# PasaLab/marlin

Measured on NVIDIA B200. Metric: fp64 dense multiply throughput (2*N^3 flop), 16384x16384 BlockMatrix 2x2 grid, higher is better.
Workload: dtype f64

## Files before the change

### include/marlin_b200.h

```cpp
#ifndef MARLIN_B200_H
#define MARLIN_B200_H

#include <stdint.h>
#include <stddef.h>

#ifdef __cplusplus
extern "C" {
#endif
#if defined(__GNUC__)
#pragma GCC visibility push(default)
#endif

#define MB_OK                 0
#define MB_ERR_INVALID_ARG   -1
#define MB_ERR_DIM_MISMATCH  -2
#define MB_ERR_UNSUPPORTED   -3
#define MB_ERR_CUDA          -4
#define MB_ERR_OOM           -5
#define MB_ERR_EMPTY         -6

typedef enum { MB_F64 = 0, MB_BF16 = 1, MB_F32 = 2 } mb_dtype;

typedef struct mb_ctx   mb_ctx;
typedef struct mb_block mb_block;
// ... 51 lines not shown
int32_t mb_block_sum(mb_ctx* ctx, const mb_block* A, double* sum_out);

int32_t mb_block_gemv(mb_ctx* ctx, const mb_block* A, const mb_block* x, mb_block* y, int32_t accumulate);
int32_t mb_block_dot(mb_ctx* ctx, const mb_block* x, const mb_block* y, double* dot_out);
int32_t mb_block_ger(mb_ctx* ctx, const mb_block* x, const mb_block* y, mb_block* out);

int32_t mb_block_lu(mb_ctx* ctx, mb_block* A, int32_t* perm_out);
int32_t mb_block_cholesky(mb_ctx* ctx, mb_block* A);
int32_t mb_block_inverse(mb_ctx* ctx, const mb_block* A, mb_block* out);
int32_t mb_block_trsm(mb_ctx* ctx, const mb_block* T, int32_t lower, int32_t unit_diagonal, mb_block* B);

int32_t mb_fill_uniform(mb_ctx* ctx, mb_block* blk, int64_t partition_seed, int64_t first,
                        double lo, double hi, int32_t row_major);
int64_t mb_hash_seed(int64_t seed);
int32_t mb_partition_seeds(int64_t seed, int32_t num_partitions, int64_t* seeds_out);

int32_t mb_choose_split(int64_t m, int64_t k, int64_t n, int32_t cores, int32_t out_mkn[3]);
int32_t mb_choose_strategy(int64_t a_rows, int64_t a_cols, int64_t b_cols, int32_t cores,
                           int32_t broadcast_threshold_mb, int32_t other_is_block,
                           int32_t* strategy, int32_t out_mkn[3]);
int32_t mb_mult_partition(int32_t i, int32_t j, int32_t kk, int32_t m, int32_t k, int32_t n);
int32_t mb_elem_partition(int32_t row, int32_t col, int32_t blks_by_col);
int32_t mb_block_len(int64_t total, int32_t parts, int32_t* block_len, int32_t* actual_parts);

int32_t mb_matmul_blocked(mb_ctx* ctx, mb_block* const* A_tiles, mb_block* const* B_tiles,
                          int32_t m, int32_t k, int32_t n, mb_block* const* C_tiles);
int32_t mb_matmul_blocked_subset(mb_ctx* ctx, mb_block* const* A_tiles, mb_block* const* B_tiles,
                                 int32_t m, int32_t k, int32_t n, mb_block* const* C_tiles,
                                 const int32_t* c_ids, int32_t num_c);

int32_t mb_matmul_blocked_host(mb_ctx* ctx, const double* const* A_host, const double* const* B_host,
                               int32_t m, int32_t k, int32_t n, const int32_t* row_len, const int32_t* k_len,
                               const int32_t* col_len, double* const* C_host);

int32_t mb_matmul_rowsharded(mb_ctx* ctx, const mb_block* A_rows, const mb_block* B, mb_block* C_rows);
int32_t mb_matmul_rowsharded_host(mb_ctx* ctx, const double* A_host, int64_t rows, int32_t k, const double* B_host,
                                  int32_t n, double* C_host);

int32_t mb_ipc_export(mb_ctx* ctx, const void* device_ptr, uint8_t handle_out[64], int64_t* offset_out,
                      int64_t* alloc_bytes_out);
int32_t mb_ipc_open(mb_ctx* ctx, const uint8_t handle[64], void** base_out);
int32_t mb_ipc_close_all(mb_ctx* ctx);
int32_t mb_flags_alloc(mb_ctx* ctx, int32_t count, void** flags_out);
int32_t mb_flags_free(mb_ctx* ctx, void* flags);
int32_t mb_flag_signal(mb_ctx* ctx, void* flag, int64_t value);
int32_t mb_flag_wait(mb_ctx* ctx, const void* flag, int64_t value);
int32_t mb_memcpy_async(mb_ctx* ctx, void* dst, const void* src, int64_t bytes);

typedef struct mb_comm mb_comm;
#define MB_ERR_TIMEOUT       -7
int32_t mb_comm_init(mb_ctx* ctx, int32_t rank, int32_t world, const char* session, mb_comm** out);
int32_t mb_comm_destroy(mb_comm* comm);
int32_t mb_comm_rank(const mb_comm* comm);
int32_t mb_comm_world(const mb_comm* comm);
int32_t mb_comm_barrier(mb_comm* comm);
int32_t mb_comm_abort(mb_comm* comm);
int32_t mb_comm_check(mb_comm* comm);
int32_t mb_dist_plan(int32_t m, int32_t k, int32_t n, int32_t world, int32_t* product_rank_out, int32_t* c_owner_out);
int32_t mb_matmul_blocked_dist(mb_comm* comm, mb_block* const* A_tiles, const int32_t* a_owner,
                               mb_block* const* B_tiles, const int32_t* b_owner, int32_t m, int32_t k, int32_t n,
                               const int32_t* row_len, const int32_t* k_len, const int32_t* col_len, int32_t dtype,
                               mb_block* const* C_tiles);

int32_t mb_dist_host_homes(int32_t m, int32_t k, int32_t n, int32_t world, int32_t* a_home, int32_t* b_home);
int32_t mb_matmul_blocked_dist_host(mb_comm* comm, const double* const* A_host, const int32_t* a_home,
                                    const double* const* B_host, const int32_t* b_home, int32_t m, int32_t k, int32_t n,
// ... 30 lines not shown
```

### marlin_b200/_native.py

```python
from __future__ import annotations

import ctypes as C
import os
from pathlib import Path

MB_OK = 0
MB_ERR_INVALID_ARG = -1
MB_ERR_DIM_MISMATCH = -2
MB_ERR_UNSUPPORTED = -3
MB_ERR_CUDA = -4
MB_ERR_OOM = -5
MB_ERR_EMPTY = -6
MB_ERR_TIMEOUT = -7

MB_F64, MB_BF16, MB_F32 = 0, 1, 2

_LIB_PATH = Path(__file__).resolve().parent / "lib" / "libmarlin_b200.so"

c_ctx = C.c_void_p
c_blk = C.c_void_p
c_sp = C.c_void_p
c_i32 = C.c_int32
c_i64 = C.c_int64
c_f64 = C.c_double
# ... 24 lines not shown
    "mb_set_fp64_mode": (c_i32, [c_ctx, c_i32, c_i32]),
    "mb_dgemm_device": (c_i32, [c_ctx, C.c_char, C.c_char, c_i32, c_i32, c_i32, c_f64, C.c_void_p, c_i32,
                                C.c_void_p, c_i32, c_f64, C.c_void_p, c_i32]),
    "mb_dgemm_device_generic": (c_i32, [c_ctx, C.c_char, C.c_char, c_i32, c_i32, c_i32, c_f64, C.c_void_p, c_i32,
                                        C.c_void_p, c_i32, c_f64, C.c_void_p, c_i32]),
    "mb_dgemm_host": (c_i32, [c_ctx, C.c_char, C.c_char, c_i32, c_i32, c_i32, c_f64, C.c_void_p, c_i64, c_i32,
                              C.c_void_p, c_i64, c_i32, c_f64, C.c_void_p, c_i64, c_i32]),
    "mb_block_add": (c_i32, [c_ctx, c_blk, c_blk, c_blk]),
    "mb_block_sub": (c_i32, [c_ctx, c_blk, c_blk, c_blk]),
    "mb_block_hadamard": (c_i32, [c_ctx, c_blk, c_blk, c_blk]),
    "mb_block_axpb": (c_i32, [c_ctx, c_blk, c_f64, c_f64, c_blk]),
    "mb_block_fill": (c_i32, [c_ctx, c_blk, c_f64]),
    "mb_block_div": (c_i32, [c_ctx, c_blk, c_f64, c_i32, c_blk]),
    "mb_block_transpose": (c_i32, [c_ctx, c_blk, c_blk]),
    "mb_block_copy": (c_i32, [c_ctx, c_blk, c_blk]),
    "mb_block_sum": (c_i32, [c_ctx, c_blk, c_dp]),
    "mb_block_gemv": (c_i32, [c_ctx, c_blk, c_blk, c_blk, c_i32]),
    "mb_block_dot": (c_i32, [c_ctx, c_blk, c_blk, c_dp]),
    "mb_block_ger": (c_i32, [c_ctx, c_blk, c_blk, c_blk]),
    "mb_block_lu": (c_i32, [c_ctx, c_blk, C.POINTER(c_i32)]),
    "mb_block_cholesky": (c_i32, [c_ctx, c_blk]),
    "mb_block_inverse": (c_i32, [c_ctx, c_blk, c_blk]),
    "mb_block_trsm": (c_i32, [c_ctx, c_blk, c_i32, c_i32, c_blk]),
    "mb_fill_uniform": (c_i32, [c_ctx, c_blk, c_i64, c_i64, c_f64, c_f64, c_i32]),
    "mb_hash_seed": (c_i64, [c_i64]),
    "mb_partition_seeds": (c_i32, [c_i64, c_i32, C.POINTER(c_i64)]),
    "mb_choose_split": (c_i32, [c_i64, c_i64, c_i64, c_i32, C.POINTER(c_i32)]),
    "mb_choose_strategy": (c_i32, [c_i64, c_i64, c_i64, c_i32, c_i32, c_i32, C.POINTER(c_i32), C.POINTER(c_i32)]),
    "mb_mult_partition": (c_i32, [c_i32, c_i32, c_i32, c_i32, c_i32, c_i32]),
    "mb_elem_partition": (c_i32, [c_i32, c_i32, c_i32]),
    "mb_block_len": (c_i32, [c_i64, c_i32, C.POINTER(c_i32), C.POINTER(c_i32)]),
    "mb_matmul_blocked_host": (c_i32, [c_ctx, C.POINTER(C.c_void_p), C.POINTER(C.c_void_p), c_i32, c_i32, c_i32,
                                       C.POINTER(c_i32), C.POINTER(c_i32), C.POINTER(c_i32), C.POINTER(C.c_void_p)]),
    "mb_matmul_rowsharded": (c_i32, [c_ctx, c_blk, c_blk, c_blk]),
    "mb_matmul_rowsharded_host": (c_i32, [c_ctx, C.c_void_p, c_i64, c_i32, C.c_void_p, c_i32, C.c_void_p]),
    "mb_ipc_export": (c_i32, [c_ctx, C.c_void_p, C.c_char_p, C.POINTER(c_i64), C.POINTER(c_i64)]),
    "mb_ipc_open": (c_i32, [c_ctx, C.c_char_p, C.POINTER(C.c_void_p)]),
    "mb_ipc_close_all": (c_i32, [c_ctx]),
    "mb_flags_alloc": (c_i32, [c_ctx, c_i32, C.POINTER(C.c_void_p)]),
    "mb_flags_free": (c_i32, [c_ctx, C.c_void_p]),
    "mb_flag_signal": (c_i32, [c_ctx, C.c_void_p, c_i64]),
    "mb_flag_wait": (c_i32, [c_ctx, C.c_void_p, c_i64]),
    "mb_memcpy_async": (c_i32, [c_ctx, C.c_void_p, C.c_void_p, c_i64]),
    "mb_matmul_blocked_subset": (c_i32, [c_ctx, C.POINTER(c_blk), C.POINTER(c_blk), c_i32, c_i32, c_i32, C.POINTER(c_blk),
                                         C.POINTER(c_i32), c_i32]),
    "mb_matmul_blocked": (c_i32, [c_ctx, C.POINTER(c_blk), C.POINTER(c_blk), c_i32, c_i32, c_i32, C.POINTER(c_blk)]),
    "mb_comm_init": (c_i32, [c_ctx, c_i32, c_i32, C.c_char_p, C.POINTER(C.c_void_p)]),
    "mb_comm_destroy": (c_i32, [C.c_void_p]),
    "mb_comm_rank": (c_i32, [C.c_void_p]),
    "mb_comm_world": (c_i32, [C.c_void_p]),
    "mb_comm_barrier": (c_i32, [C.c_void_p]),
    "mb_comm_check": (c_i32, [C.c_void_p]),
    "mb_comm_abort": (c_i32, [C.c_void_p]),
    "mb_dist_plan": (c_i32, [c_i32, c_i32, c_i32, c_i32, C.POINTER(c_i32), C.POINTER(c_i32)]),
    "mb_dist_host_homes": (c_i32, [c_i32, c_i32, c_i32, c_i32, C.POINTER(c_i32), C.POINTER(c_i32)]),
    "mb_matmul_blocked_dist_host": (c_i32, [C.c_void_p, C.POINTER(C.c_void_p), C.POINTER(c_i32), C.POINTER(C.c_void_p), C.POINTER(c_i32),
                                            c_i32, c_i32, c_i32, C.POINTER(c_i32), C.POINTER(c_i32), C.POINTER(c_i32), C.POINTER(C.c_void_p)]),
    "mb_host_alloc_shared": (c_i32, [C.c_char_p, c_i64, C.POINTER(C.c_void_p)]),
    "mb_host_free_shared": (c_i32, [C.c_char_p, C.c_void_p, c_i64, c_i32]),
    "mb_matmul_blocked_dist": (c_i32, [C.c_void_p, C.POINTER(c_blk), C.POINTER(c_i32), C.POINTER(c_blk), C.POINTER(c_i32), c_i32, c_i32,
                                       c_i32, C.POINTER(c_i32), C.POINTER(c_i32), C.POINTER(c_i32), c_i32, C.POINTER(c_blk)]),
    "mb_csc_check": (c_i32, [c_i32, c_i32, C.POINTER(c_i32), C.POINTER(c_i32)]),
    "mb_spblock_upload": (c_i32, [c_ctx, c_i32, c_i32, C.POINTER(c_i32), C.POINTER(c_i32), c_dp, C.POINTER(c_sp)]),
    "mb_spblock_download": (c_i32, [c_ctx, c_sp, C.POINTER(c_i32), C.POINTER(c_i32), c_dp]),
    "mb_spblock_info": (c_i32, [c_sp, C.POINTER(c_i32), C.POINTER(c_i32), C.POINTER(c_i64)]),
    "mb_spblock_free": (c_i32, [c_ctx, c_sp]),
    "mb_spblock_copy": (c_i32, [c_ctx, c_sp, C.POINTER(c_sp)]),
# ... 59 lines not shown
```

### marlin_b200/csrc/capi.cu

```cuda
#include "../../include/marlin_b200.h"
#include "elementwise.h"
#include "gemm_f64.h"
#include "gemm_bf16.h"
#include "gemm_ozaki.h"
#include "blas12.h"
#include "factor.h"
#include "sparse.h"

#include <cuda_runtime.h>
#include <algorithm>
#include <cstdarg>
#include <cstdlib>
#include <cstdio>
#include <cstring>
#include <new>
#include <atomic>
#include <mutex>
#include <vector>

#include "internal.h"

namespace {

thread_local char g_err[512] = "";
// ... 126 lines not shown
    MB_CUDA(cudaGetDeviceProperties(&prop, device));
    if (prop.major != 10)
        return fail(MB_ERR_UNSUPPORTED, "mb_init: device %d is sm_%d%d; this library is built for sm_100a only", device,
                    prop.major, prop.minor);
    mb_ctx* ctx = new (std::nothrow) mb_ctx();
    if (!ctx) return fail(MB_ERR_OOM, "host allocation failed");
    ctx->device = device;
    ctx->num_sms = prop.multiProcessorCount;
    MB_CUDA(cudaStreamCreateWithFlags(&ctx->own_stream, cudaStreamNonBlocking));
    ctx->stream = ctx->own_stream;
    MB_CUDA(cudaMalloc(&ctx->scratch, sizeof(double) * std::max(mb::sum_scratch_doubles(), mb::dot_scratch_doubles())));
    MB_CUDA(cudaMallocHost(&ctx->host_scalar, sizeof(double)));
    MB_CUDA(cudaEventCreate(&ctx->ev0));
    MB_CUDA(cudaEventCreate(&ctx->ev1));
    *out = ctx;
    return MB_OK;
}

int32_t mb_shutdown(mb_ctx* ctx) {
    if (!ctx) return MB_OK;
    cudaSetDevice(ctx->device);
    cudaStreamSynchronize(ctx->stream);
    if (ctx->scratch) cudaFree(ctx->scratch);
    if (ctx->vec_ws) cudaFree(ctx->vec_ws);
    if (ctx->int_ws) cudaFree(ctx->int_ws);
    if (ctx->int_host) cudaFreeHost(ctx->int_host);
    if (ctx->host_scalar) cudaFreeHost(ctx->host_scalar);
    if (ctx->ev0) cudaEventDestroy(ctx->ev0);
    if (ctx->ev1) cudaEventDestroy(ctx->ev1);
    if (ctx->own_stream) cudaStreamDestroy(ctx->own_stream);
    if (ctx->h2d_stream) cudaStreamDestroy(ctx->h2d_stream);
    if (ctx->d2h_stream) cudaStreamDestroy(ctx->d2h_stream);
    if (ctx->workspace) cudaFree(ctx->workspace);
    if (ctx->ozaki_ws) cudaFree(ctx->ozaki_ws);
    delete ctx;
    return MB_OK;
}

int32_t mb_set_stream(mb_ctx* ctx, void* cuda_stream) {
    if (!ctx) return fail(MB_ERR_INVALID_ARG, "null context");
    ctx->stream = static_cast<cudaStream_t>(cuda_stream);
    return MB_OK;
}

int32_t mb_reset_stream(mb_ctx* ctx) {
    if (!ctx) return fail(MB_ERR_INVALID_ARG, "null context");
    ctx->stream = ctx->own_stream;
    return MB_OK;
}

int32_t mb_synchronize(mb_ctx* ctx) {
    MB_CTX(ctx);
    MB_CUDA(cudaStreamSynchronize(ctx->stream));
    return MB_OK;
}

int64_t mb_launch_count(mb_ctx* ctx) { return ctx ? (int64_t)ctx->launches.load() : 0; }

int32_t mb_timer_start(mb_ctx* ctx) {
    MB_CTX(ctx);
    MB_LOCK(ctx);
    MB_CUDA(cudaEventRecord(ctx->ev0, ctx->stream));
    return MB_OK;
}
int32_t mb_timer_stop(mb_ctx* ctx, float* ms_out) {
    MB_CTX(ctx);
// ... 368 lines not shown
                    ++group; ns = 0; in_group = 0;
                };
                for (int kk = 0; kk < k && e == cudaSuccess; ++kk)
                    for (int k0 = 0; k0 < Ks[kk] && e == cudaSuccess;) {
                        const int len = (int)std::min<long long>(Ks[kk] - k0, kchain - in_group);
                        sa[ns] = static_cast<const char*>(Ap[kk]) + (size_t)k0 * la[kk] * 2;
                        sb[ns] = static_cast<const char*>(Bp[kk]) + (size_t)k0 * 2;
                        sla[ns] = la[kk]; slb[ns] = lb[kk]; sk[ns] = len;
                        ++ns; in_group += len; k0 += len;
                        if (in_group >= kchain || ns == 8) flush();
                    }
                flush();
            }
            if (e == cudaSuccess) { ctx->launches += launches; continue; }
            if (e != cudaErrorNotSupported) return cuda_fail(e, "gemm_bf16_segments");
            cudaGetLastError();
        }
        for (int kk = 0; kk < k; ++kk) {
            int32_t r = mb_block_gemm(ctx, A_tiles[i * k + kk], B_tiles[kk * n + j], C_tiles[id], kk > 0);
            if (r) return r;
        }
    }
    return MB_OK;
}

int32_t mb_matmul_blocked(mb_ctx* ctx, mb_block* const* A_tiles, mb_block* const* B_tiles, int32_t m, int32_t k,
                          int32_t n, mb_block* const* C_tiles) {
    if (m <= 0 || k <= 0 || n <= 0) return fail(MB_ERR_INVALID_ARG, "mb_matmul_blocked: bad argument");
    std::vector<int32_t> ids(m * n);
    for (int c = 0; c < m * n; ++c) ids[c] = c;
    return mb_matmul_blocked_subset(ctx, A_tiles, B_tiles, m, k, n, C_tiles, ids.data(), m * n);
}

int32_t mb_matmul_blocked_host(mb_ctx* ctx, const double* const* A_host, const double* const* B_host, int32_t m,
                               int32_t k, int32_t n, const int32_t* row_len, const int32_t* k_len, const int32_t* col_len,
                               double* const* C_host) {
    MB_CTX(ctx);
    MB_LOCK(ctx);
    if (!A_host || !B_host || !C_host || !row_len || !k_len || !col_len || m <= 0 || k <= 0 || n <= 0)
        return fail(MB_ERR_INVALID_ARG, "mb_matmul_blocked_host: bad argument");
    if (!ctx->h2d_stream) {
        MB_CUDA(cudaStreamCreateWithFlags(&ctx->h2d_stream, cudaStreamNonBlocking));
        MB_CUDA(cudaStreamCreateWithFlags(&ctx->d2h_stream, cudaStreamNonBlocking));
    }
    auto even = [](int x) { return (x + 1) & ~1; };
    auto slot = [](size_t bytes) { return (bytes + 255) & ~size_t(255); };
    std::vector<size_t> offA(m * k), offB(k * n), offC(m * n);
    size_t total = 0;
    for (int i = 0; i < m; ++i)
        for (int kk = 0; kk < k; ++kk) { offA[i * k + kk] = total; total += slot((size_t)even(row_len[i]) * k_len[kk] * 8); }
    for (int kk = 0; kk < k; ++kk)
        for (int j = 0; j < n; ++j) { offB[kk * n + j] = total; total += slot((size_t)even(k_len[kk]) * col_len[j] * 8); }
    for (int i = 0; i < m; ++i)
        for (int j = 0; j < n; ++j) { offC[i * n + j] = total; total += slot((size_t)even(row_len[i]) * col_len[j] * 8); }
    if (total > ctx->workspace_bytes) {
        if (ctx->workspace) { MB_CUDA(cudaDeviceSynchronize()); cudaFree(ctx->workspace); ctx->workspace = nullptr; ctx->workspace_bytes = 0; }
        MB_CUDA(cudaMalloc(&ctx->workspace, total));
        ctx->workspace_bytes = total;
    }
    char* base = static_cast<char*>(ctx->workspace);
    std::vector<cudaEvent_t> evA(m * k, nullptr), evB(k * n, nullptr), evC(m * n, nullptr);
    cudaEvent_t ev_start = nullptr, ev_done = nullptr;
    int32_t rc = MB_OK;
    cudaError_t e = cudaSuccess;
    auto upload = [&](bool isA, int idx, int rows, int cols, const double* host, size_t off, cudaEvent_t& ev) {
        if (ev || e != cudaSuccess) return;
        e = cudaEventCreateWithFlags(&ev, cudaEventDisableTiming);
        if (e != cudaSuccess) return;
        if (rows > 0 && cols > 0)
            e = cudaMemcpy2DAsync(base + off, (size_t)even(rows) * 8, host, (size_t)rows * 8, (size_t)rows * 8, cols,
                                  cudaMemcpyHostToDevice, ctx->h2d_stream);
        if (e == cudaSuccess) e = cudaEventRecord(ev, ctx->h2d_stream);
        (void)isA; (void)idx;
    };
    e = cudaEventCreateWithFlags(&ev_start, cudaEventDisableTiming);
    if (e == cudaSuccess) e = cudaEventRecord(ev_start, ctx->stream);
    if (e == cudaSuccess) e = cudaStreamWaitEvent(ctx->h2d_stream, ev_start, 0);
    auto gemm_cols = [&](int i, int j, int kk, int c0, int c1) {
        const int lda8 = even(row_len[i]) > 0 ? even(row_len[i]) : 1, ldb8 = even(k_len[kk]) > 0 ? even(k_len[kk]) : 1;
        rc = dgemm_device_impl(ctx, 'N', 'N', row_len[i], c1 - c0, k_len[kk], 1.0, reinterpret_cast<double*>(base + offA[i * k + kk]), lda8,
                               reinterpret_cast<double*>(base + offB[kk * n + j]) + (size_t)c0 * ldb8, ldb8, kk > 0 ? 1.0 : 0.0,
                               reinterpret_cast<double*>(base + offC[i * n + j]) + (size_t)c0 * lda8, lda8, false);
    };
    std::vector<cudaEvent_t> chunk_events;
    for (int i = 0; i < m && e == cudaSuccess && rc == MB_OK; ++i)
        for (int j = 0; j < n && e == cudaSuccess && rc == MB_OK; ++j) {
            for (int kk = 0; kk < k && e == cudaSuccess && rc == MB_OK; ++kk) {
                const bool first_product = (i == 0 && j == 0 && kk == 0);
                const bool last_product = (i == m - 1 && j == n - 1 && kk == k - 1);
                if (first_product && !last_product && k_len[kk] >= 1024 && row_len[i] > 0 && col_len[j] > 0) {
                    const int nk = 4;
                    const int lda8 = even(row_len[i]), ldb8 = even(k_len[kk]);
                    for (int q = 0; q < nk && e == cudaSuccess && rc == MB_OK; ++q) {
                        const int k0 = q == 0 ? 0 : (int)(((long long)k_len[kk] * q / nk) & ~15ll);
                        const int k1 = q == nk - 1 ? k_len[kk] : (int)(((long long)k_len[kk] * (q + 1) / nk) & ~15ll);
                        cudaEvent_t ev = nullptr;
                        e = cudaEventCreateWithFlags(&ev, cudaEventDisableTiming);
                        if (e != cudaSuccess) break;
                        chunk_events.push_back(ev);
                        e = cudaMemcpy2DAsync(base + offA[i * k + kk] + (size_t)k0 * lda8 * 8, (size_t)lda8 * 8,
                                              A_host[i * k + kk] + (size_t)k0 * row_len[i], (size_t)row_len[i] * 8,
                                              (size_t)row_len[i] * 8, k1 - k0, cudaMemcpyHostToDevice, ctx->h2d_stream);
                        if (e == cudaSuccess)
                            e = cudaMemcpy2DAsync(base + offB[kk * n + j] + (size_t)k0 * 8, (size_t)ldb8 * 8, B_host[kk * n + j] + k0,
                                                  (size_t)k_len[kk] * 8, (size_t)(k1 - k0) * 8, col_len[j], cudaMemcpyHostToDevice,
                                                  ctx->h2d_stream);
                        if (e == cudaSuccess) e = cudaEventRecord(ev, ctx->h2d_stream);
                        if (e == cudaSuccess) e = cudaStreamWaitEvent(ctx->stream, ev, 0);
                        if (e != cudaSuccess) break;
                        rc = dgemm_device_impl(ctx, 'N', 'N', row_len[i], col_len[j], k1 - k0, 1.0,
                                               reinterpret_cast<double*>(base + offA[i * k + kk]) + (size_t)k0 * lda8, lda8,
                                               reinterpret_cast<double*>(base + offB[kk * n + j]) + k0, ldb8, (kk > 0 || q > 0) ? 1.0 : 0.0,
                                               reinterpret_cast<double*>(base + offC[i * n + j]), lda8, false);
                    }
                    if (e != cudaSuccess || rc != MB_OK) break;
                    e = cudaEventCreateWithFlags(&evA[i * k + kk], cudaEventDisableTiming);
                    if (e == cudaSuccess) e = cudaEventRecord(evA[i * k + kk], ctx->h2d_stream);
                    if (e == cudaSuccess) e = cudaEventCreateWithFlags(&evB[kk * n + j], cudaEventDisableTiming);
                    if (e == cudaSuccess) e = cudaEventRecord(evB[kk * n + j], ctx->h2d_stream);
                    continue;
                }
                const int nch = ((first_product || last_product) && col_len[j] >= 1024) ? 4 : 1;
                upload(true, i * k + kk, row_len[i], k_len[kk], A_host[i * k + kk], offA[i * k + kk], evA[i * k + kk]);
                if (e != cudaSuccess) break;
                e = cudaStreamWaitEvent(ctx->stream, evA[i * k + kk], 0);
                if (e != cudaSuccess) break;
                if (nch == 1) {
                    upload(false, kk * n + j, k_len[kk], col_len[j], B_host[kk * n + j], offB[kk * n + j], evB[kk * n + j]);
                    if (e == cudaSuccess) e = cudaStreamWaitEvent(ctx->stream, evB[kk * n + j], 0);
                    if (e != cudaSuccess) break;
                    gemm_cols(i, j, kk, 0, col_len[j]);
                    continue;
                }
                const bool b_pending = (evB[kk * n + j] == nullptr);
                const int ldb8 = even(k_len[kk]), ldc8 = even(row_len[i]);
                for (int q = 0; q < nch && e == cudaSuccess && rc == MB_OK; ++q) {
                    const int c0 = (int)((long long)col_len[j] * q / nch), c1 = (int)((long long)col_len[j] * (q + 1) / nch);
                    if (b_pending) {
                        cudaEvent_t ev = nullptr;
                        e = cudaEventCreateWithFlags(&ev, cudaEventDisableTiming);
                        if (e != cudaSuccess) break;
                        chunk_events.push_back(ev);
                        e = cudaMemcpy2DAsync(base + offB[kk * n + j] + (size_t)c0 * ldb8 * 8, (size_t)ldb8 * 8,
                                              B_host[kk * n + j] + (size_t)c0 * k_len[kk], (size_t)k_len[kk] * 8, (size_t)k_len[kk] * 8,
                                              c1 - c0, cudaMemcpyHostToDevice, ctx->h2d_stream);
                        if (e == cudaSuccess) e = cudaEventRecord(ev, ctx->h2d_stream);
                        if (e == cudaSuccess) e = cudaStreamWaitEvent(ctx->stream, ev, 0);
                        if (e != cudaSuccess) break;
                        if (q == nch - 1) {
                            e = cudaEventCreateWithFlags(&evB[kk * n + j], cudaEventDisableTiming);
                            if (e == cudaSuccess) e = cudaEventRecord(evB[kk * n + j], ctx->h2d_stream);
                        }
                    } else if (q == 0) {
                        e = cudaStreamWaitEvent(ctx->stream, evB[kk * n + j], 0);
                    }
                    if (e != cudaSuccess) break;
                    gemm_cols(i, j, kk, c0, c1);
                    if (rc != MB_OK) break;
                    if (last_product) {
                        cudaEvent_t ev = nullptr;
                        e = cudaEventCreateWithFlags(&ev, cudaEventDisableTiming);
                        if (e != cudaSuccess) break;
                        chunk_events.push_back(ev);
                        e = cudaEventRecord(ev, ctx->stream);
                        if (e == cudaSuccess) e = cudaStreamWaitEvent(ctx->d2h_stream, ev, 0);
                        if (e == cudaSuccess && row_len[i] > 0 && c1 > c0)
                            e = cudaMemcpy2DAsync(C_host[i * n + j] + (size_t)c0 * row_len[i], (size_t)row_len[i] * 8,
                                                  base + offC[i * n + j] + (size_t)c0 * ldc8 * 8, (size_t)ldc8 * 8, (size_t)row_len[i] * 8,
                                                  c1 - c0, cudaMemcpyDeviceToHost, ctx->d2h_stream);
                    }
                }
            }
            if (e != cudaSuccess || rc != MB_OK) break;
            const bool chunked_out = (i == m - 1 && j == n - 1 && col_len[j] >= 1024);
            if (chunked_out) continue;
            e = cudaEventCreateWithFlags(&evC[i * n + j], cudaEventDisableTiming);
            if (e == cudaSuccess) e = cudaEventRecord(evC[i * n + j], ctx->stream);
            if (e == cudaSuccess) e = cudaStreamWaitEvent(ctx->d2h_stream, evC[i * n + j], 0);
            if (e == cudaSuccess && row_len[i] > 0 && col_len[j] > 0)
                e = cudaMemcpy2DAsync(C_host[i * n + j], (size_t)row_len[i] * 8, base + offC[i * n + j], (size_t)even(row_len[i]) * 8,
                                      (size_t)row_len[i] * 8, col_len[j], cudaMemcpyDeviceToHost, ctx->d2h_stream);
        }
    if (e == cudaSuccess && rc == MB_OK) {
        e = cudaEventCreateWithFlags(&ev_done, cudaEventDisableTiming);
        if (e == cudaSuccess) e = cudaEventRecord(ev_done, ctx->d2h_stream);
        if (e == cudaSuccess) e = cudaStreamWaitEvent(ctx->stream, ev_done, 0);
        if (e == cudaSuccess) e = cudaStreamSynchronize(ctx->d2h_stream);
    } else {
        cudaStreamSynchronize(ctx->h2d_stream); cudaStreamSynchronize(ctx->stream); cudaStreamSynchronize(ctx->d2h_stream);
    }
    for (auto ev : evA) if (ev) cudaEventDestroy(ev);
    for (auto ev : evB) if (ev) cudaEventDestroy(ev);
    for (auto ev : evC) if (ev) cudaEventDestroy(ev);
    for (auto ev : chunk_events) if (ev) cudaEventDestroy(ev);
    if (ev_start) cudaEventDestroy(ev_start);
    if (ev_done) cudaEventDestroy(ev_done);
    if (rc != MB_OK) return rc;
    if (e != cudaSuccess) return cuda_fail(e, "mb_matmul_blocked_host");
    return MB_OK;
}

int32_t mb_matmul_rowsharded(mb_ctx* ctx, const mb_block* A_rows, const mb_block* B, mb_block* C_rows) {
    MB_CTX(ctx);
    if (!A_rows || !B || !C_rows) return fail(MB_ERR_INVALID_ARG, "mb_matmul_rowsharded: null block");
    if (A_rows->cols != B->rows)
        return fail(MB_ERR_DIM_MISMATCH, "Dimension mismatch during matrix-matrix multiplication: %d vs %d", A_rows->cols, B->rows);
    return mb_block_gemm(ctx, A_rows, B, C_rows, 0);
}

int32_t mb_matmul_rowsharded_host(mb_ctx* ctx, const double* A_host, int64_t rows, int32_t k, const double* B_host,
                                  int32_t n, double* C_host) {
    MB_CTX(ctx);
    MB_LOCK(ctx);
    if (rows < 0 || k < 0 || n < 0 || (rows > 0 && ((k > 0 && !A_host) || (n > 0 && !C_host))) || (k > 0 && n > 0 && !B_host))
        return fail(MB_ERR_INVALID_ARG, "mb_matmul_rowsharded_host: bad argument");
    if (rows == 0 || n == 0) return MB_OK;
    if (!ctx->h2d_stream) {
        MB_CUDA(cudaStreamCreateWithFlags(&ctx->h2d_stream, cudaStreamNonBlocking));
        MB_CUDA(cudaStreamCreateWithFlags(&ctx->d2h_stream, cudaStreamNonBlocking));
    }
    constexpr int SLOTS = 3;
    long long chunk_mib = 256;
    if (const char* ev = getenv("MARLIN_B200_ROWSHARD_CHUNK_MIB")) chunk_mib = std::max(1, atoi(ev));
    long long chunk = (chunk_mib << 20) / (8ll * std::max(std::max(k, n), 1));
    chunk = std::max(128ll, chunk / 128 * 128);
    chunk = std::min<long long>(chunk, (rows + 127) / 128 * 128);
    const int kk = std::max(k, 1);
    auto slot = [](size_t bytes) { return (bytes + 255) & ~size_t(255); };
    const size_t bytesB = slot((size_t)kk * n * 8), bytesA = slot((size_t)chunk * kk * 8), bytesC = slot((size_t)chunk * n * 8);
// ... 527 lines not shown
```

### marlin_b200/csrc/internal.h

```cpp
#pragma once
#include "../../include/marlin_b200.h"

#include <cuda_runtime.h>
#include <atomic>
#include <cstdarg>
#include <cstdio>
#include <mutex>

struct mb_ctx {
    int device = 0;
    int num_sms = 148;
    cudaStream_t own_stream = nullptr;
    cudaStream_t stream = nullptr;
    std::atomic<long long> launches{0};
    double* scratch = nullptr;
    double* host_scalar = nullptr;
    cudaEvent_t ev0 = nullptr, ev1 = nullptr;
    cudaStream_t h2d_stream = nullptr, d2h_stream = nullptr;
    void* workspace = nullptr;
    size_t workspace_bytes = 0;
    int fp64_mode = MB_FP64_NATIVE;
    int fp64_slices = 7;
    int fp64_bits = 7;
    void* ozaki_ws = nullptr;
    size_t ozaki_ws_bytes = 0;
    double* vec_ws = nullptr;
    size_t vec_ws_doubles = 0;
    int* int_ws = nullptr;
    size_t int_ws_count = 0;
    int* int_host = nullptr;
    size_t int_host_count = 0;
    std::recursive_mutex mu;
};

struct mb_block {
    void* data = nullptr;
    long long offset = 0;
    int rows = 0, cols = 0;
    int ld = 0;
    int is_transpose = 0;
    int dtype = MB_F64;
    int owns = 0;
    int device = 0;
    void* ready_event = nullptr;
};

struct mb_spblock {
    int rows = 0, cols = 0;
    long long nnz = 0;
    int* col_ptr = nullptr;
    int* row_idx = nullptr;
    double* val = nullptr;
    int device = 0;
// ... 49 lines not shown
```

Baseline: 36.41.

## Reorder host blocked matmul k-outer and overlap the last tile's download with compute

The host-staged blocked multiply now walks products k-outer (kk, i, j) through a helper that also reports tile upload order. The first product is pipelined in growing k-chunks, and the second product splits its newly needed operand into row or column bands so upload and compute overlap. The final product runs as a grouped GEMM whose column bands signal device flags, so the D2H copy of each band can start as soon as that band is finished. This aims to hide PCIe transfer time at both ends, at the cost of more complex stream and flag synchronisation and a persistent flag buffer.

```diff
diff --git a/include/marlin_b200.h b/include/marlin_b200.h
--- a/include/marlin_b200.h
+++ b/include/marlin_b200.h
@@ -107,6 +107,7 @@
 int32_t mb_matmul_blocked_host(mb_ctx* ctx, const double* const* A_host, const double* const* B_host,
                                int32_t m, int32_t k, int32_t n, const int32_t* row_len, const int32_t* k_len,
                                const int32_t* col_len, double* const* C_host);
+int32_t mb_blocked_host_order(int32_t m, int32_t k, int32_t n, int32_t* seq, int32_t* uploads);
 
 int32_t mb_matmul_rowsharded(mb_ctx* ctx, const mb_block* A_rows, const mb_block* B, mb_block* C_rows);
 int32_t mb_matmul_rowsharded_host(mb_ctx* ctx, const double* A_host, int64_t rows, int32_t k, const double* B_host,
diff --git a/marlin_b200/_native.py b/marlin_b200/_native.py
--- a/marlin_b200/_native.py
+++ b/marlin_b200/_native.py
@@ -80,7 +80,8 @@
     "mb_block_len": (c_i32, [c_i64, c_i32, C.POINTER(c_i32), C.POINTER(c_i32)]),
     "mb_matmul_blocked_host": (c_i32, [c_ctx, C.POINTER(C.c_void_p), C.POINTER(C.c_void_p), c_i32, c_i32, c_i32,
                                        C.POINTER(c_i32), C.POINTER(c_i32), C.POINTER(c_i32), C.POINTER(C.c_void_p)]),
-    "mb_matmul_rowsharded": (c_i32, [c_ctx, c_blk, c_blk, c_blk]),
+    "mb_blocked_host_order": (c_i32, [c_i32, c_i32, c_i32, C.POINTER(c_i32), C.POINTER(c_i32)]),
+    "mb_matmul_rowsharded":(c_i32, [c_ctx, c_blk, c_blk, c_blk]),
     "mb_matmul_rowsharded_host": (c_i32, [c_ctx, C.c_void_p, c_i64, c_i32, C.c_void_p, c_i32, C.c_void_p]),
     "mb_ipc_export": (c_i32, [c_ctx, C.c_void_p, C.c_char_p, C.POINTER(c_i64), C.POINTER(c_i64)]),
     "mb_ipc_open": (c_i32, [c_ctx, C.c_char_p, C.POINTER(C.c_void_p)]),
diff --git a/marlin_b200/csrc/capi.cu b/marlin_b200/csrc/capi.cu
--- a/marlin_b200/csrc/capi.cu
+++ b/marlin_b200/csrc/capi.cu
@@ -182,6 +182,7 @@
     if (ctx->h2d_stream) cudaStreamDestroy(ctx->h2d_stream);
     if (ctx->d2h_stream) cudaStreamDestroy(ctx->d2h_stream);
     if (ctx->workspace) cudaFree(ctx->workspace);
+    if (ctx->host_flags) cudaFree(ctx->host_flags);
     if (ctx->ozaki_ws) cudaFree(ctx->ozaki_ws);
     delete ctx;
     return MB_OK;
@@ -616,6 +617,23 @@
     return mb_matmul_blocked_subset(ctx, A_tiles, B_tiles, m, k, n, C_tiles, ids.data(), m * n);
 }
 
+int32_t mb_blocked_host_order(int32_t m, int32_t k, int32_t n, int32_t* seq, int32_t* uploads) {
+    if (m <= 0 || k <= 0 || n <= 0 || !seq) return fail(MB_ERR_INVALID_ARG, "mb_blocked_host_order: bad argument");
+    std::vector<char> seen((size_t)m * k + (size_t)k * n, 0);
+    int p = 0, u = 0;
+    for (int kk = 0; kk < k; ++kk)
+        for (int i = 0; i < m; ++i)
+            for (int j = 0; j < n; ++j) {
+                seq[p++] = i * n * k + j * k + kk;
+                for (int t : {i * k + kk, m * k + kk * n + j})
+                    if (!seen[t]) {
+                        seen[t] = 1;
+                        if (uploads) uploads[u++] = t;
+                    }
+            }
+    return MB_OK;
+}
+
 int32_t mb_matmul_blocked_host(mb_ctx* ctx, const double* const* A_host, const double* const* B_host, int32_t m,
                                int32_t k, int32_t n, const int32_t* row_len, const int32_t* k_len, const int32_t* col_len,
                                double* const* C_host) {
@@ -628,6 +646,7 @@
         MB_CUDA(cudaStreamCreateWithFlags(&ctx->d2h_stream, cudaStreamNonBlocking));
     }
     auto even = [](int x) { return (x + 1) & ~1; };
+    auto ld8 = [&](int rows) { return std::max(even(rows), 1); };
     auto slot = [](size_t bytes) { return (bytes + 255) & ~size_t(255); };
     std::vector<size_t> offA(m * k), offB(k * n), offC(m * n);
     size_t total = 0;
@@ -642,143 +661,139 @@
         MB_CUDA(cudaMalloc(&ctx->workspace, total));
         ctx->workspace_bytes = total;
     }
+    const int na = m * k, np = m * k * n;
+    std::vector<int32_t> seq(np);
+    int32_t rc = mb_blocked_host_order(m, k, n, seq.data(), nullptr);
+    if (rc != MB_OK) return rc;
+    const int last = seq[np - 1], li = last / (n * k), lj = (last / k) % n, lkk = last % k;
+    const bool banded_last = ctx->fp64_mode == MB_FP64_NATIVE && col_len[lj] >= 1024 && row_len[li] > 0 && k_len[lkk] > 0;
+    if (banded_last && !ctx->host_flags) {
+        MB_CUDA(cudaMalloc(&ctx->host_flags, 2 * mb::G2_MAX_ENTRIES * sizeof(unsigned long long)));
+        MB_CUDA(cudaMemset(ctx->host_flags, 0, 2 * mb::G2_MAX_ENTRIES * sizeof(unsigned long long)));
+    }
     char* base = static_cast<char*>(ctx->workspace);
-    std::vector<cudaEvent_t> evA(m * k, nullptr), evB(k * n, nullptr), evC(m * n, nullptr);
-    cudaEvent_t ev_start = nullptr, ev_done = nullptr;
-    int32_t rc = MB_OK;
     cudaError_t e = cudaSuccess;
-    auto upload = [&](bool isA, int idx, int rows, int cols, const double* host, size_t off, cudaEvent_t& ev) {
-        if (ev || e != cudaSuccess) return;
-        e = cudaEventCreateWithFlags(&ev, cudaEventDisableTiming);
-        if (e != cudaSuccess) return;
-        if (rows > 0 && cols > 0)
-            e = cudaMemcpy2DAsync(base + off, (size_t)even(rows) * 8, host, (size_t)rows * 8, (size_t)rows * 8, cols,
-                                  cudaMemcpyHostToDevice, ctx->h2d_stream);
-        if (e == cudaSuccess) e = cudaEventRecord(ev, ctx->h2d_stream);
-        (void)isA; (void)idx;
+    std::vector<cudaEvent_t> events;
+    std::vector<cudaEvent_t> ev_tile(na + k * n, nullptr);
+    auto mark = [&](cudaStream_t s) -> cudaEvent_t {
+        cudaEvent_t ev = nullptr;
+        if (e == cudaSuccess) e = cudaEventCreateWithFlags(&ev, cudaEventDisableTiming);
+        if (e != cudaSuccess) return nullptr;
+        events.push_back(ev);
+        e = cudaEventRecord(ev, s);
+        return ev;
     };
-    e = cudaEventCreateWithFlags(&ev_start, cudaEventDisableTiming);
-    if (e == cudaSuccess) e = cudaEventRecord(ev_start, ctx->stream);
-    if (e == cudaSuccess) e = cudaStreamWaitEvent(ctx->h2d_stream, ev_start, 0);
-    auto gemm_cols = [&](int i, int j, int kk, int c0, int c1) {
-        const int lda8 = even(row_len[i]) > 0 ? even(row_len[i]) : 1, ldb8 = even(k_len[kk]) > 0 ? even(k_len[kk]) : 1;
-        rc = dgemm_device_impl(ctx, 'N', 'N', row_len[i], c1 - c0, k_len[kk], 1.0, reinterpret_cast<double*>(base + offA[i * k + kk]), lda8,
-                               reinterpret_cast<double*>(base + offB[kk * n + j]) + (size_t)c0 * ldb8, ldb8, kk > 0 ? 1.0 : 0.0,
-                               reinterpret_cast<double*>(base + offC[i * n + j]) + (size_t)c0 * lda8, lda8, false);
+    auto after = [&](cudaStream_t s, cudaEvent_t ev) {
+        if (e == cudaSuccess && ev) e = cudaStreamWaitEvent(s, ev, 0);
     };
-    std::vector<cudaEvent_t> chunk_events;
-    for (int i = 0; i < m && e == cudaSuccess && rc == MB_OK; ++i)
-        for (int j = 0; j < n && e == cudaSuccess && rc == MB_OK; ++j) {
-            for (int kk = 0; kk < k && e == cudaSuccess && rc == MB_OK; ++kk) {
-                const bool first_product = (i == 0 && j == 0 && kk == 0);
-                const bool last_product = (i == m - 1 && j == n - 1 && kk == k - 1);
-                if (first_product && !last_product && k_len[kk] >= 1024 && row_len[i] > 0 && col_len[j] > 0) {
-                    const int nk = 4;
-                    const int lda8 = even(row_len[i]), ldb8 = even(k_len[kk]);
-                    for (int q = 0; q < nk && e == cudaSuccess && rc == MB_OK; ++q) {
-                        const int k0 = q == 0 ? 0 : (int)(((long long)k_len[kk] * q / nk) & ~15ll);
-                        const int k1 = q == nk - 1 ? k_len[kk] : (int)(((long long)k_len[kk] * (q + 1) / nk) & ~15ll);
-                        cudaEvent_t ev = nullptr;
-                        e = cudaEventCreateWithFlags(&ev, cudaEventDisableTiming);
-                        if (e != cudaSuccess) break;
-                        chunk_events.push_back(ev);
-                        e = cudaMemcpy2DAsync(base + offA[i * k + kk] + (size_t)k0 * lda8 * 8, (size_t)lda8 * 8,
-                                              A_host[i * k + kk] + (size_t)k0 * row_len[i], (size_t)row_len[i] * 8,
-                                              (size_t)row_len[i] * 8, k1 - k0, cudaMemcpyHostToDevice, ctx->h2d_stream);
-                        if (e == cudaSuccess)
-                            e = cudaMemcpy2DAsync(base + offB[kk * n + j] + (size_t)k0 * 8, (size_t)ldb8 * 8, B_host[kk * n + j] + k0,
-                                                  (size_t)k_len[kk] * 8, (size_t)(k1 - k0) * 8, col_len[j], cudaMemcpyHostToDevice,
-                                                  ctx->h2d_stream);
-                        if (e == cudaSuccess) e = cudaEventRecord(ev, ctx->h2d_stream);
-                        if (e == cudaSuccess) e = cudaStreamWaitEvent(ctx->stream, ev, 0);
-                        if (e != cudaSuccess) break;
-                        rc = dgemm_device_impl(ctx, 'N', 'N', row_len[i], col_len[j], k1 - k0, 1.0,
-                                               reinterpret_cast<double*>(base + offA[i * k + kk]) + (size_t)k0 * lda8, lda8,
-                                               reinterpret_cast<double*>(base + offB[kk * n + j]) + k0, ldb8, (kk > 0 || q > 0) ? 1.0 : 0.0,
-                                               reinterpret_cast<double*>(base + offC[i * n + j]), lda8, false);
-                    }
-                    if (e != cudaSuccess || rc != MB_OK) break;
-                    e = cudaEventCreateWithFlags(&evA[i * k + kk], cudaEventDisableTiming);
-                    if (e == cudaSuccess) e = cudaEventRecord(evA[i * k + kk], ctx->h2d_stream);
-                    if (e == cudaSuccess) e = cudaEventCreateWithFlags(&evB[kk * n + j], cudaEventDisableTiming);
-                    if (e == cudaSuccess) e = cudaEventRecord(evB[kk * n + j], ctx->h2d_stream);
-                    continue;
+    struct Tile { const double* host; int rows, cols; char* dev; };
+    auto operand = [&](int t) -> Tile {
+        if (t < na) return {A_host[t], row_len[t / k], k_len[t % k], base + offA[t]};
+        const int b = t - na;
+        return {B_host[b], k_len[b / n], col_len[b % n], base + offB[b]};
+    };
+    auto h2d = [&](const Tile& T, int r0, int r1, int c0, int c1) {
+        if (e != cudaSuccess || r1 <= r0 || c1 <= c0) return;
+        const size_t ldd = ld8(T.rows);
+        e = cudaMemcpy2DAsync(T.dev + ((size_t)c0 * ldd + r0) * 8, ldd * 8, T.host + (size_t)c0 * T.rows + r0,
+                              (size_t)T.rows * 8, (size_t)(r1 - r0) * 8, c1 - c0, cudaMemcpyHostToDevice, ctx->h2d_stream);
+    };
+    auto d2h = [&](int i, int j, int c0, int c1) {
+        const int rows = row_len[i];
+        if (e != cudaSuccess || rows <= 0 || c1 <= c0) return;
+        const size_t ldd = ld8(rows);
+        e = cudaMemcpy2DAsync(C_host[i * n + j] + (size_t)c0 * rows, (size_t)rows * 8, base + offC[i * n + j] + (size_t)c0 * ldd * 8,
+                              ldd * 8, (size_t)rows * 8, c1 - c0, cudaMemcpyDeviceToHost, ctx->d2h_stream);
+    };
+    auto gemm = [&](int i, int j, int kk, int r0, int r1, int c0, int c1, int k0, int k1, bool accumulate) {
+        if (e != cudaSuccess || rc != MB_OK) return;
+        const int lda = ld8(row_len[i]), ldb = ld8(k_len[kk]);
+        rc = dgemm_device_impl(ctx, 'N', 'N', r1 - r0, c1 - c0, k1 - k0, 1.0,
+                               reinterpret_cast<const double*>(base + offA[i * k + kk]) + (size_t)k0 * lda + r0, lda,
+                               reinterpret_cast<const double*>(base + offB[kk * n + j]) + (size_t)c0 * ldb + k0, ldb,
+                               accumulate ? 1.0 : 0.0, reinterpret_cast<double*>(base + offC[i * n + j]) + (size_t)c0 * lda + r0,
+                               lda, false);
+    };
+    after(ctx->h2d_stream, mark(ctx->stream));
+    std::vector<char> sent(na + k * n, 0);
+    for (int p = 0; p < np && e == cudaSuccess && rc == MB_OK; ++p) {
+        const int s = seq[p], i = s / (n * k), j = (s / k) % n, kk = s % k;
+        const int tA = i * k + kk, tB = na + kk * n + j;
+        const Tile TA = operand(tA), TB = operand(tB);
+        const int M = row_len[i], N = col_len[j], K = k_len[kk];
+        const bool newA = !sent[tA], newB = !sent[tB];
+        sent[tA] = sent[tB] = 1;
+        const bool is_last = p == np - 1;
+        if (p == 0 && !is_last && K >= 1024 && M > 0 && N > 0) {
+            for (int k0 = 0, k1; k0 < K && e == cudaSuccess && rc == MB_OK; k0 = k1) {
+                k1 = std::min(K, (256 + k0 + k0 / 4) & ~15);
+                if (K - k1 < 256) k1 = K;
+                h2d(TA, 0, M, k0, k1);
+                h2d(TB, k0, k1, 0, N);
+                after(ctx->stream, mark(ctx->h2d_stream));
+                gemm(i, j, kk, 0, M, 0, N, k0, k1, kk > 0 || k0 > 0);
+            }
+            ev_tile[tA] = ev_tile[tB] = mark(ctx->h2d_stream);
+        } else if (p == 1 && !is_last && newA != newB && (newA ? M : N) >= 1024) {
+            after(ctx->stream, ev_tile[newA ? tB : tA]);
+            const int ext = newA ? M : N;
+            for (int q = 0; q < 4 && e == cudaSuccess && rc == MB_OK; ++q) {
+                const int b0 = (int)(((long long)ext * q / 4) & ~127ll), b1 = q == 3 ? ext : (int)(((long long)ext * (q + 1) / 4) & ~127ll);
+                if (newA) h2d(TA, b0, b1, 0, K); else h2d(TB, 0, K, b0, b1);
+                after(ctx->stream, mark(ctx->h2d_stream));
+                if (newA) gemm(i, j, kk, b0, b1, 0, N, 0, K, kk > 0); else gemm(i, j, kk, 0, M, b0, b1, 0, K, kk > 0);
+            }
+            ev_tile[newA ? tA : tB] = mark(ctx->h2d_stream);
+        } else {
+            if (newA) { h2d(TA, 0, TA.rows, 0, TA.cols); ev_tile[tA] = mark(ctx->h2d_stream); }
+            if (newB) { h2d(TB, 0, TB.rows, 0, TB.cols); ev_tile[tB] = mark(ctx->h2d_stream); }
+            after(ctx->stream, ev_tile[tA]);
+            after(ctx->stream, ev_tile[tB]);
+            if (is_last && banded_last) {
+                if (e != cudaSuccess || rc != MB_OK) break;
+                const unsigned long long epoch = ++ctx->host_epoch;
+                unsigned long long *ctr = ctx->host_flags, *sig = ctx->host_flags + mb::G2_MAX_ENTRIES;
+                const int lda = ld8(M), ldb = ld8(K);
+                double* Cd = reinterpret_cast<double*>(base + offC[i * n + j]);
+                static thread_local mb::G2Launch L;
+                L = mb::G2Launch();
+                L.na = L.nb = 1;
+                L.A[0].ptr = reinterpret_cast<const double*>(TA.dev); L.A[0].ld = lda; L.A[0].rows = M; L.A[0].cols = K;
+                L.B[0].ptr = reinterpret_cast<const double*>(TB.dev); L.B[0].ld = ldb; L.B[0].rows = K; L.B[0].cols = N;
+                const int w = ((N + 15) / 16 + 127) & ~127;
+                for (int c0 = 0; c0 < N; c0 += w) {
+                    mb::G2Entry& en = L.E[L.ne];
+                    en.nseg = 1;
+                    en.n_off = c0; en.M = M; en.N = std::min(w, N - c0);
+                    en.D = Cd + (size_t)c0 * lda; en.ldd = lda;
+                    if (kk > 0) { en.Cin = en.D; en.ldcin = lda; }
+                    en.done_ctr = ctr + L.ne; en.sig_local = sig + L.ne; en.sig_val = epoch;
+                    ++L.ne;
                 }
-                const int nch = ((first_product || last_product) && col_len[j] >= 1024) ? 4 : 1;
-                upload(true, i * k + kk, row_len[i], k_len[kk], A_host[i * k + kk], offA[i * k + kk], evA[i * k + kk]);
-                if (e != cudaSuccess) break;
-                e = cudaStreamWaitEvent(ctx->stream, evA[i * k + kk], 0);
-                if (e != cudaSuccess) break;
-                if (nch == 1) {
-                    upload(false, kk * n + j, k_len[kk], col_len[j], B_host[kk * n + j], offB[kk * n + j], evB[kk * n + j]);
-                    if (e == cudaSuccess) e = cudaStreamWaitEvent(ctx->stream, evB[kk * n + j], 0);
-                    if (e != cudaSuccess) break;
-                    gemm_cols(i, j, kk, 0, col_len[j]);
-                    continue;
+                e = cudaMemsetAsync(ctr, 0, L.ne * sizeof(unsigned long long), ctx->stream);
+                int launches = 0;
+                if (e == cudaSuccess) e = mb::gemm_f64_grouped2(L, ctx->num_sms, ctx->stream, &launches);
+                ctx->launches += launches;
+                for (int b = 0; b < L.ne && e == cudaSuccess; ++b) {
+                    e = mb::stream_wait64_geq(sig + b, epoch, ctx->d2h_stream);
+                    d2h(i, j, L.E[b].n_off, L.E[b].n_off + L.E[b].N);
                 }
-                const bool b_pending = (evB[kk * n + j] == nullptr);
-                const int ldb8 = even(k_len[kk]), ldc8 = even(row_len[i]);
-                for (int q = 0; q < nch && e == cudaSuccess && rc == MB_OK; ++q) {
-                    const int c0 = (int)((long long)col_len[j] * q / nch), c1 = (int)((long long)col_len[j] * (q + 1) / nch);
-                    if (b_pending) {
-                        cudaEvent_t ev = nullptr;
-                        e = cudaEventCreateWithFlags(&ev, cudaEventDisableTiming);
-                        if (e != cudaSuccess) break;
-                        chunk_events.push_back(ev);
-                        e = cudaMemcpy2DAsync(base + offB[kk * n + j] + (size_t)c0 * ldb8 * 8, (size_t)ldb8 * 8,
-                                              B_host[kk * n + j] + (size_t)c0 * k_len[kk], (size_t)k_len[kk] * 8, (size_t)k_len[kk] * 8,
-                                              c1 - c0, cudaMemcpyHostToDevice, ctx->h2d_stream);
-                        if (e == cudaSuccess) e = cudaEventRecord(ev, ctx->h2d_stream);
-                        if (e == cudaSuccess) e = cudaStreamWaitEvent(ctx->stream, ev, 0);
-                        if (e != cudaSuccess) break;
-                        if (q == nch - 1) {
-                            e = cudaEventCreateWithFlags(&evB[kk * n + j], cudaEventDisableTiming);
-                            if (e == cudaSuccess) e = cudaEventRecord(evB[kk * n + j], ctx->h2d_stream);
-                        }
-                    } else if (q == 0) {
-                        e = cudaStreamWaitEvent(ctx->stream, evB[kk * n + j], 0);
-                    }
-                    if (e != cudaSuccess) break;
-                    gemm_cols(i, j, kk, c0, c1);
-                    if (rc != MB_OK) break;
-                    if (last_product) {
-                        cudaEvent_t ev = nullptr;
-                        e = cudaEventCreateWithFlags(&ev, cudaEventDisableTiming);
-                        if (e != cudaSuccess) break;
-                        chunk_events.push_back(ev);
-                        e = cudaEventRecord(ev, ctx->stream);
-                        if (e == cudaSuccess) e = cudaStreamWaitEvent(ctx->d2h_stream, ev, 0);
-                        if (e == cudaSuccess && row_len[i] > 0 && c1 > c0)
-                            e = cudaMemcpy2DAsync(C_host[i * n + j] + (size_t)c0 * row_len[i], (size_t)row_len[i] * 8,
-                                                  base + offC[i * n + j] + (size_t)c0 * ldc8 * 8, (size_t)ldc8 * 8, (size_t)row_len[i] * 8,
-                                                  c1 - c0, cudaMemcpyDeviceToHost, ctx->d2h_stream);
-                    }
-                }
+                continue;
             }
-            if (e != cudaSuccess || rc != MB_OK) break;
-            const bool chunked_out = (i == m - 1 && j == n - 1 && col_len[j] >= 1024);
-            if (chunked_out) continue;
-            e = cudaEventCreateWithFlags(&evC[i * n + j], cudaEventDisableTiming);
-            if (e == cudaSuccess) e = cudaEventRecord(evC[i * n + j], ctx->stream);
-            if (e == cudaSuccess) e = cudaStreamWaitEvent(ctx->d2h_stream, evC[i * n + j], 0);
-            if (e == cudaSuccess && row_len[i] > 0 && col_len[j] > 0)
-                e = cudaMemcpy2DAsync(C_host[i * n + j], (size_t)row_len[i] * 8, base + offC[i * n + j], (size_t)even(row_len[i]) * 8,
-                                      (size_t)row_len[i] * 8, col_len[j], cudaMemcpyDeviceToHost, ctx->d2h_stream);
+            gemm(i, j, kk, 0, M, 0, N, 0, K, kk > 0);
         }
+        if (kk == k - 1) {
+            after(ctx->d2h_stream, mark(ctx->stream));
+            d2h(i, j, 0, N);
+        }
+    }
     if (e == cudaSuccess && rc == MB_OK) {
-        e = cudaEventCreateWithFlags(&ev_done, cudaEventDisableTiming);
-        if (e == cudaSuccess) e = cudaEventRecord(ev_done, ctx->d2h_stream);
-        if (e == cudaSuccess) e = cudaStreamWaitEvent(ctx->stream, ev_done, 0);
+        after(ctx->stream, mark(ctx->d2h_stream));
         if (e == cudaSuccess) e = cudaStreamSynchronize(ctx->d2h_stream);
     } else {
         cudaStreamSynchronize(ctx->h2d_stream); cudaStreamSynchronize(ctx->stream); cudaStreamSynchronize(ctx->d2h_stream);
     }
-    for (auto ev : evA) if (ev) cudaEventDestroy(ev);
-    for (auto ev : evB) if (ev) cudaEventDestroy(ev);
-    for (auto ev : evC) if (ev) cudaEventDestroy(ev);
-    for (auto ev : chunk_events) if (ev) cudaEventDestroy(ev);
-    if (ev_start) cudaEventDestroy(ev_start);
-    if (ev_done) cudaEventDestroy(ev_done);
+    for (auto ev : events) cudaEventDestroy(ev);
     if (rc != MB_OK) return rc;
     if (e != cudaSuccess) return cuda_fail(e, "mb_matmul_blocked_host");
     return MB_OK;
diff --git a/marlin_b200/csrc/internal.h b/marlin_b200/csrc/internal.h
--- a/marlin_b200/csrc/internal.h
+++ b/marlin_b200/csrc/internal.h
@@ -19,6 +19,8 @@
     cudaStream_t h2d_stream = nullptr, d2h_stream = nullptr;
     void* workspace = nullptr;
     size_t workspace_bytes = 0;
+    unsigned long long* host_flags = nullptr;
+    unsigned long long host_epoch = 0;
     int fp64_mode = MB_FP64_NATIVE;
     int fp64_slices = 7;
     int fp64_bits = 7;
```

Result: no change. 36.41 (median of 6 runs) (+0.0%).
